# SludgePhD/Compeg

Hardware: AMD Instinct MI355X
Metric: Mpixels/s decoded (4K 4:2:2 restart-interval baseline JPEG -> RGBA8 in HBM) (higher is better)
Workload: dtype u32 bit-reader / i16 levels / f32 IDCT / u8 RGBA

## Files before the change

### compeg_amd/csrc/runtime.cpp

```cpp
#include "runtime.h"
#include "lab.h"

#include <hip/hip_runtime.h>

#include <algorithm>
#include <chrono>
#include <string>
#include <cstdio>
#include <cstdlib>
#include <condition_variable>
#include <cstring>
#include <mutex>
#include <thread>

namespace compeg {

Status hip_status(hipError_t e, const char *what)
{
    if (e == hipSuccess)
        return Status{};
    char buf[256];
    snprintf(buf, sizeof buf, "%s: %s", what, hipGetErrorString(e));
    return Status::error(COMPEG_E_HIP, buf);
}
// ... 323 lines not shown
}

}

}

using namespace compeg;

compeg_decoder::compeg_decoder() : scan(pinned_alloc, pinned_free)
{
    const unsigned hw = std::thread::hardware_concurrency();
    unsigned threads = hw >= 32 ? 8 : (hw >= 8 ? 4 : 1);
    bool asked = false;
    if (const char *e = getenv("COMPEG_SCAN_THREADS")) {
        threads = unsigned(std::max(1, std::min(16, atoi(e))));
        asked = true;
    }
    scan.set_threads(threads, !asked);
}

compeg_decoder::~compeg_decoder()
{
    if (last_stream || upload_pending)
        (void)hipStreamSynchronize(last_stream);
    if (upload_done)
        (void)hipEventDestroy(upload_done);
    if (decode_done)
        (void)hipEventDestroy(decode_done);
    if (gpu)
        compeg_gpu_release(gpu);
}

Status compeg_decoder::preprocess_on_device(const ImageData &img, hipStream_t stream, uint32_t &nwords,
                                            uint32_t &nstarts, uint32_t &span, bool &fell_back, size_t blob_bytes,
                                            const BlobWriter &before_submit)
{
    fell_back = false;
    if (img.scan_len > 0xfffffff0u) {
        fell_back = true;
        return Status{};
    }
    const uint32_t len = uint32_t(img.scan_len), expected = img.metadata.total_restart_intervals;
    uint32_t slots = 1;
    while (slots < expected)
        slots <<= 1;
    const uint32_t ntiles = scan_tiles(len);
    size_t total = 64;
    auto take = [&](size_t bytes) {
        const size_t at = total;
        total += align_up(bytes, 256);
        return at;
    };
    const size_t o_res = 0, o_desc = take(sizeof(ScanDesc)), o_blob = take(before_submit ? blob_bytes : 0),
                 o_raw = take(size_t(len) + 64), o_ts = take(size_t(ntiles) * kScanTileStateBytes + 32),
                 o_st = take(size_t(slots) * 4), o_w = take(size_t(len) + len / 3 + 64);
    CG_TRY(scan_arena.reserve(total + kStreamSlackBytes));
    CG_TRY(raw_stage.reserve(o_raw + len + 64));
    uint8_t *da = static_cast<uint8_t *>(scan_arena.ptr), *hs = static_cast<uint8_t *>(raw_stage.ptr);
    ScanDesc s;
    s.raw = da + o_raw;
    s.len = len;
    s.ntiles = ntiles;
    s.slots = slots;
    s.tile_state = reinterpret_cast<uint32_t *>(da + o_ts);
    s.starts_out = reinterpret_cast<uint32_t *>(da + o_st);
    s.words_out = da + o_w;
    s.result = reinterpret_cast<uint32_t *>(da + o_res);
    dev_words = da + o_w;
    dev_starts = da + o_st;
    EnqueueTrace trace;
    memset(hs, 0, o_blob);
    if (before_submit)
        CG_TRY(before_submit(hs + o_blob, da + o_blob, &s.patch_nwords, &s.patch_nstarts));
    memcpy(hs + o_desc, &s, sizeof s);
    const size_t piece = scan.threads() > 1 ? size_t(len) + 1 : size_t(640u << 10);
    for (size_t at = 0; at < len || at == 0; at += piece) {
        const size_t n = std::min<size_t>(piece, len - at);
        scan.copy(hs + o_raw + at, img.scan_data() + at, n);
        const size_t from = at ? o_raw + at : 0;
        if (pull_copies())
            CG_HIP(launch_pull(da + from, hs + from, o_raw + at + n - from, stream));
        else
            CG_HIP(hipMemcpyAsync(da + from, hs + from, o_raw + at + n - from, hipMemcpyHostToDevice, stream));
        if (len == 0)
            break;
    }
    trace.mark("  stage_and_copy");
    CG_HIP(launch_scan(reinterpret_cast<const ScanDesc *>(da + o_desc), 1, ntiles, stream));
    CG_TRY(scan_result.reserve(16));
    uint32_t *res = static_cast<uint32_t *>(scan_result.ptr);
    scan_result_dev = da + o_res;
    deferred_expected = expected;
    if (!before_submit)
        CG_HIP(hipMemcpyAsync(res, scan_result_dev, 16, hipMemcpyDeviceToHost, stream));
    trace.mark("submit");
    if (before_submit) {
        const uint64_t most_words = (uint64_t(len) + 3u * uint64_t(expected)) / 4u + 1u;
        const uint64_t avg = expected ? (most_words + expected - 1) / expected : most_words;
        span = uint32_t(std::min<uint64_t>(2 * avg * kWave + 64, 0x7fffffffu));
        nwords = nstarts = 0;
        deferred_check = true;
        return Status{};
    }
    CG_HIP(hipStreamSynchronize(stream));
    trace.mark("sync");
    CG_TRY(check_scan_result(fell_back));
    if (fell_back)
        return Status{};
    nwords = res[2];
    nstarts = std::min(res[0], slots);
    const uint64_t avg = expected ? (uint64_t(nwords) + expected - 1) / expected : nwords;
    span = uint32_t(std::min<uint64_t>(2 * avg * kWave + 64, 0x7fffffffu));
    return Status{};
}

Status compeg_decoder::check_scan_result(bool &fell_back)
{
    const uint32_t *res = static_cast<const uint32_t *>(scan_result.ptr);
    fell_back = (res[3] & 1u) != 0u;
    if (!fell_back && res[0] != deferred_expected) {
        char msg[128];
        snprintf(msg, sizeof msg, "restart interval count mismatch: counted %u, expected %u", res[0],
                 deferred_expected);
        warning = msg;
    }
    return Status{};
}

Status compeg_decoder::finish_deferred(const ImageData &img, hipStream_t stream)
{
    if (!deferred_check)
        return Status{};
    deferred_check = false;
    bool fell_back = false;
    CG_TRY(check_scan_result(fell_back));
    if (!fell_back)
        return Status{};
    const bool keep = device_preprocess;
    device_preprocess = false;
    Status st = enqueue(img, stream, nullptr, false);
    device_preprocess = keep;
    CG_TRY(st);
    CG_HIP(hipStreamSynchronize(stream));
    return Status{};
}

Status compeg_decoder::enqueue(const ImageData &img, hipStream_t stream, bool *changed, bool may_defer)
{
    EnqueueTrace trace;
    const auto t_enter = std::chrono::steady_clock::now();
    stage_times = compeg_stage_times{0.0, 0.0, 0.0};
    double preprocess_us = 0.0;
    struct Closer {
        compeg_decoder *self;
        std::chrono::steady_clock::time_point t0;
        const double *pre;
        ~Closer()
        {
            self->stage_times.preprocess_us = *pre;
            self->stage_times.enqueue_writes_us = EnqueueTrace::us_since(t0) - *pre;
        }
    } closer{this, t_enter, &preprocess_us};
    CG_HIP(hipSetDevice(gpu->device));
    warning.clear();

    if (!decode_done)
        CG_HIP(hipEventCreateWithFlags(&decode_done, hipEventDisableTiming));
    if (decode_pending && stream != last_stream)
        CG_HIP(hipStreamWaitEvent(stream, decode_done, 0));

    bool realloc_out = false;
    if (img.width > out_w || img.height > out_h || !out.ptr) {
// ... 260 lines not shown
            CG_TRY(ensure_walk_tables());
            CG_HIP(launch_coop_422(reinterpret_cast<const ImageDesc *>(db), 1, md.total_restart_intervals, coop, stream));
            last_kernel = COMPEG_KERNEL_COOP_TEAM;
        } else if (use_stream_kernel(plan, md.total_restart_intervals, 1)) {
            const uint64_t mcus = std::max<uint64_t>(1u, uint64_t(md.total_restart_intervals) * std::max(1u, uint32_t(md.restart_interval)));
            const StreamPlan sp = plan_stream(md.total_restart_intervals, 1, staged_lut_entries(img),
                                              uint32_t((img.scan_len / 4u + mcus - 1u) / mcus), true);
            CG_HIP(launch_fused_stream(reinterpret_cast<const ImageDesc *>(db), 1, md.total_restart_intervals, sp, stream));
            last_kernel = COMPEG_KERNEL_FUSED_STREAM;
        } else if (use_pair_kernel(md.total_restart_intervals, 1)) {
            CG_HIP(launch_pair_422(reinterpret_cast<const ImageDesc *>(db), 1, md.total_restart_intervals,
                                   plan, stream));
            last_kernel = COMPEG_KERNEL_PAIR;
        } else {
            CG_HIP(launch_fused_422(reinterpret_cast<const ImageDesc *>(db), 1, md.total_restart_intervals,
                                    plan, stream, false, md.restart_interval == 1u));
            last_kernel = COMPEG_KERNEL_FUSED;
        }
        coefficients_valid = false;
    } else {
        last_kernel = COMPEG_KERNEL_SPLIT;
        CG_HIP(launch_entropy(reinterpret_cast<const ImageDesc *>(db), 1, md.total_restart_intervals,
                              plan, stream));
        CG_HIP(launch_idct_composite(reinterpret_cast<const ImageDesc *>(db), 1, total_dus, stream));
        coefficients_valid = true;
    }
    if (deferred_check)
        CG_HIP(hipMemcpyAsync(scan_result.ptr, scan_result_dev, 16, hipMemcpyDeviceToHost, stream));
    if (!may_defer) {
        CG_HIP(hipEventRecord(decode_done, stream));
        decode_pending = true;
    }
    trace.mark("launch");
    return Status{};
}

Status compeg::ScanBuffer::process_on_gpu(compeg_gpu *gpu, const uint8_t *scan, size_t len,
                                          uint32_t expected)
{
    if (len > 0xfffffff0u)
        return Status::error(COMPEG_E_INVALID_ARG, "scan segment too large");
    CG_HIP(hipSetDevice(gpu->device));
    uint32_t slots = 1;
    while (slots < expected)
        slots <<= 1;
    const uint32_t ntiles = scan_tiles(uint32_t(len));
    DeviceBuffer arena, descbuf;
    size_t total = 64;
    auto take = [&](size_t bytes) {
        const size_t at = total;
        total += align_up(bytes, 256);
        return at;
    };
    const size_t o_raw = take(len + 64), o_ts = take(size_t(ntiles) * kScanTileStateBytes + 32),
                 o_st = take(size_t(slots) * 4), o_w = take(len + len / 3 + 64), o_res = take(kScanResultBytes);
    CG_TRY(arena.reserve(total));
    CG_TRY(descbuf.reserve(sizeof(ScanDesc)));
    uint8_t *da = static_cast<uint8_t *>(arena.ptr);
    CG_HIP(hipMemset(da, 0, total));
    if (len)
        CG_HIP(hipMemcpy(da + o_raw, scan, len, hipMemcpyHostToDevice));
    ScanDesc s;
    s.raw = da + o_raw;
    s.len = uint32_t(len);
    s.ntiles = ntiles;
    s.slots = slots;
    s.tile_state = reinterpret_cast<uint32_t *>(da + o_ts);
    s.starts_out = reinterpret_cast<uint32_t *>(da + o_st);
    s.words_out = da + o_w;
    s.result = reinterpret_cast<uint32_t *>(da + o_res);
    CG_HIP(hipMemcpy(descbuf.ptr, &s, sizeof s, hipMemcpyHostToDevice));
    CG_HIP(launch_scan(static_cast<const ScanDesc *>(descbuf.ptr), 1, ntiles, gpu->stream));
    CG_HIP(hipStreamSynchronize(gpu->stream));
    uint32_t res[4];
    CG_HIP(hipMemcpy(res, da + o_res, 16, hipMemcpyDeviceToHost));
    if (res[3] & 1u)
        return process(scan, len, expected);
    const size_t out_cap = ((len + len / 3 + 3) / 4) * 4;
    if (!words_.reserve(out_cap + 8) || !starts_.reserve(size_t(slots) * 4))
        return Status::error(COMPEG_E_HIP, "out of host memory in ScanBuffer");
    nwords_ = res[2];
    nstarts_ = std::min(res[0], slots);
    if (nwords_)
        CG_HIP(hipMemcpy(words_.data, da + o_w, nwords_ * 4, hipMemcpyDeviceToHost));
    if (nstarts_)
        CG_HIP(hipMemcpy(starts_.data, da + o_st, nstarts_ * 4, hipMemcpyDeviceToHost));
    if (res[0] != expected) {
        char msg[128];
        snprintf(msg, sizeof msg, "restart interval count mismatch: counted %u, expected %u", res[0], expected);
        return Status::error(COMPEG_E_COUNT_MISMATCH, msg);
    }
    return Status{};
}

hipError_t shared_copy_streams(int device, std::vector<hipStream_t> &out)
{
    static std::mutex m;
    static std::vector<hipStream_t> pool[64];
    std::lock_guard<std::mutex> lock(m);
    if (device < 0 || device >= 64)
        return hipErrorInvalidDevice;
    while (pool[device].size() < 4) {
        hipStream_t c = nullptr;
        const hipError_t e = hipStreamCreateWithFlags(&c, hipStreamNonBlocking);
        if (e != hipSuccess)
            return e;
        pool[device].push_back(c);
    }
    out = pool[device];
    return hipSuccess;
}

compeg_batch::~compeg_batch()
{
    (void)hipStreamSynchronize(last_stream);
    if (gpu)
        (void)hipStreamSynchronize(gpu->stream);
    for (hipStream_t c : copy_streams)
        (void)hipStreamSynchronize(c);
    for (hipEvent_t e : events)
        (void)hipEventDestroy(e);
    if (decode_done)
        (void)hipEventDestroy(decode_done);
    if (gpu)
        compeg_gpu_release(gpu);
}

namespace {

constexpr const char *kLayoutBoundExceeded = "layout bound exceeded";
// ... 492 lines not shown
        const uint8_t *host;
        size_t bytes, dev;
    };
    std::vector<Run> runs;
    std::vector<size_t> run_of(n, 0);
    for (size_t i = 0; i < n; i++) {
        bool joins = false;
        if (!runs.empty() && pinned[i] && pinned[i - 1]) {
            const Run &r = runs.back();
            const uint8_t *end = r.host + r.bytes;
            const bool one_allocation = alloc[i].base && alloc[i].base == alloc[i - 1].base && alloc[i].end == alloc[i - 1].end &&
                                        src[i].bytes + src[i].len <= alloc[i].end && r.host >= alloc[i].base;
            joins = group_of(i) == group_of(r.first) && src[i].bytes >= end && size_t(src[i].bytes - end) <= kMaxGap &&
                    (src[i].bytes == end || one_allocation) && size_t(src[i].bytes - r.host) + src[i].len <= kMaxRunBytes;
        }
        if (joins) {
            runs.back().last = i;
            runs.back().bytes = size_t(src[i].bytes - runs.back().host) + src[i].len;
        } else {
            runs.push_back(Run{i, i, src[i].bytes, src[i].len, 0});
        }
        run_of[i] = runs.size() - 1;
    }

    struct Layout {
        size_t sent, tables, tile_state, starts, words;
        size_t staged;
        size_t tile_cap, slot_cap;
    };
    std::vector<Layout> lay(n);
    size_t total = 0;
    auto take = [&](size_t bytes) {
        const size_t at = total;
        total += align_up(bytes, 256);
        return at;
    };
    const size_t o_results = take(n * kScanResultBytes);
    constexpr size_t kUnparsedTablesCap = size_t(32) << 10;
    size_t tables_bytes = 0;
    for (size_t i = 0; i < n; i++) {
        lay[i].tables = tables_bytes;
        tables_bytes += align_up(given ? table_blob_bytes(*given[i]) : kUnparsedTablesCap, 256);
    }
    const size_t o_tables = take(tables_bytes);
    size_t staged_total = align_up(tables_bytes, 256);
    for (Run &r : runs)
        r.dev = take(64 + align_up(r.bytes + 64, 16)) + 64;
    for (size_t i = 0; i < n; i++) {
        Layout &L = lay[i];
        const size_t len = src[i].len;
        L.tables += o_tables;
        L.sent = runs[run_of[i]].dev + size_t(src[i].bytes - runs[run_of[i]].host);
        L.tile_cap = scan_tiles(uint32_t(len));
        L.tile_state = take(L.tile_cap * kScanTileStateBytes + 32);
        L.slot_cap = ScanBuffer::start_slots(src[i].intervals);
        L.starts = take(L.slot_cap * 4);
        L.words = take(len + len / 3 + 64);
        L.staged = staged_total;
        staged_total += align_up(len + 64, 256);
    }
    CG_TRY(scan_arena.reserve(total + kStreamSlackBytes));
    CG_TRY(scan_descs.reserve(n * sizeof(ScanDesc) + 256));
    hipStream_t st = gpu->stream;
    CG_TRY(dev_descs.reserve(n * sizeof(ImageDesc) + 256));
    CG_HIP(shared_copy_streams(gpu->device, copy_streams));
    uint8_t *da = static_cast<uint8_t *>(scan_arena.ptr);
    CG_HIP(hipMemsetAsync(da + o_results, 0, n * kScanResultBytes, st));
    CG_TRY(stage.reserve((any_pageable ? staged_total : align_up(tables_bytes, 256)) + 256));
    uint8_t *hs = static_cast<uint8_t *>(stage.ptr);
    const double t_layout = ms_since();

    std::vector<std::atomic<uint8_t>> staged_ready(n), parsed_ready(n);
    for (size_t i = 0; i < n; i++) {
        staged_ready[i].store(pinned[i], std::memory_order_relaxed);
        parsed_ready[i].store(given ? 1 : 0, std::memory_order_relaxed);
    }
    unsigned nthreads = threads > 0 ? unsigned(threads) : std::min(16u, std::max(1u, std::thread::hardware_concurrency()));
    nthreads = unsigned(std::min<size_t>(nthreads, std::max<size_t>(n, 1)));
    std::atomic<size_t> next_image{0};
    std::atomic<int> hip_error{int(hipSuccess)};
    std::atomic<bool> failed{false};
    std::vector<Status> results(n);
    const int device = gpu->device;
    auto prepare_images = [&] {
        for (;;) {
            const size_t i = next_image.fetch_add(1, std::memory_order_relaxed);
            if (i >= n)
                return;
            if (!given) {
                images[i] = parse(i, results[i]);
                if (!images[i] || table_blob_bytes(*images[i]) > kUnparsedTablesCap) {
                    if (images[i] && results[i].ok())
                        results[i] = Status::error(COMPEG_E_INVALID_ARG, kLayoutBoundExceeded);
                    images[i] = nullptr;
                    failed.store(true, std::memory_order_relaxed);
                }
                parsed_ready[i].store(1, std::memory_order_release);
            }
            if (!pinned[i]) {
                memcpy(hs + lay[i].staged, src[i].bytes, src[i].len);
                staged_ready[i].store(1, std::memory_order_release);
            }
            if (images[i])
                write_tables(hs + (lay[i].tables - o_tables), *images[i]);
        }
    };
    std::vector<ScanDesc> sd(n);
// ... 140 lines not shown
        CG_HIP(hipMemcpyAsync(res.data(), da + o_results, n * kScanResultBytes, hipMemcpyDeviceToHost, st));

        max_tiles = 0;
        max_intervals = max_dus = max_l2 = max_span = 0;
        algorithmic_bytes = pixels = 0;
        size_t out_total = 0;
        bool all_covered = true;
        for (size_t i = 0; i < n; i++) {
            const ImageData &img = *images[i];
            out_total += align_up(output_bytes(img.width, img.height), 256);
            max_tiles = std::max(max_tiles, sd[i].ntiles);
            max_intervals = std::max(max_intervals, img.metadata.total_restart_intervals);
            max_dus = std::max(max_dus, img.total_dus());
            max_l2 = std::max<uint32_t>(max_l2, staged_lut_entries(img));
            pixels += uint64_t(img.width) * img.height;
            all_covered = all_covered && item_of(img).covered;
        }
        note_batch_properties(images.data(), n);
        size_t ac_total = 0, dc_total = 0;
        for (size_t i = 0; i < n && generic_layout; i++) {
            ac_total += size_t(images[i]->total_dus()) * kRetained * 2;
            dc_total += size_t(images[i]->total_dus()) * 4;
        }
        if (generic_layout) {
            CG_TRY(ac.reserve(ac_total + 256));
            CG_TRY(dc.reserve(dc_total + 256));
        }
        bool fresh_out = false;
        CG_TRY(out.reserve(out_total + 256, &fresh_out));
        if (fresh_out || !all_covered)
            CG_HIP(hipMemsetAsync(out.ptr, 0, out.capacity, st));
        CG_HIP(hipStreamSynchronize(st));
        const double t_arrived = ms_since();
        last_stream = st;

        descs.assign(n, ImageDesc{});
        out_offset.assign(n, 0);
        host_fallbacks = 0;
        size_t out_at = 0, ac_at = 0, dc_at = 0;
        for (size_t i = 0; i < n; i++) {
            const Layout &L = lay[i];
            const uint32_t *r = &res[i * (kScanResultBytes / 4)];
            uint32_t nwords = r[2], nstarts = std::min(r[0], sd[i].slots), span = r[4];
            const bool ends_earlier = (r[3] & 2u) != 0u && images[i]->scan_end_deferred;
            if (ends_earlier) {
                Status ps;
                const ImageData *again = reparse ? reparse(i, ps) : nullptr;
                if (!again)
                    return ps.ok() ? Status::error(COMPEG_E_MALFORMED, "entropy-coded segment ends early") : ps;
                images[i] = again;
            }
            const ImageData &img = *images[i];
            const uint32_t expected = img.metadata.total_restart_intervals;
            if ((r[3] & 1u) || ends_earlier) {
                ScanBuffer sb;
                Status s = sb.process(img.scan_data(), img.scan_len, expected);
                if (!s.ok() && s.code != COMPEG_E_COUNT_MISMATCH)
                    return s;
                nwords = uint32_t(sb.nwords());
                nstarts = uint32_t(sb.nstarts());
                if (nwords)
                    CG_HIP(hipMemcpy(da + L.words, sb.words(), size_t(nwords) * 4, hipMemcpyHostToDevice));
                if (nstarts)
                    CG_HIP(hipMemcpy(da + L.starts, sb.starts(), size_t(nstarts) * 4, hipMemcpyHostToDevice));
                span = max_wave_span(sb.starts(), nstarts, nwords, expected);
                host_fallbacks++;
            }
            ImageDesc &d = descs[i];
            fill_desc(img, d);
            d.l1 = reinterpret_cast<const uint16_t *>(da + L.tables);
            d.l2 = reinterpret_cast<const uint16_t *>(da + L.tables + COMPEG_HUFFMAN_L1_BYTES);
            d.words = reinterpret_cast<const uint32_t *>(da + L.words);
            d.starts = reinterpret_cast<const uint32_t *>(da + L.starts);
            d.nwords = nwords;
            d.nstarts = nstarts;
            d.ac = generic_layout ? reinterpret_cast<int16_t *>(static_cast<uint8_t *>(ac.ptr) + ac_at) : nullptr;
            d.dc = generic_layout ? reinterpret_cast<int32_t *>(static_cast<uint8_t *>(dc.ptr) + dc_at) : nullptr;
            ac_at += size_t(img.total_dus()) * kRetained * 2;
            dc_at += size_t(img.total_dus()) * 4;
            out_offset[i] = out_at;
            d.out = static_cast<uint8_t *>(out.ptr) + out_at;
            out_at += align_up(output_bytes(img.width, img.height), 256);
            d.out_w = img.width;
            d.out_h = img.height;
            d.out_pitch = output_pitch(img.width);
            d.out_alloc_h = output_rows(img.height);
            max_span = std::max(max_span, span);
            if (i == 0) {
                coop_r = img.metadata.restart_interval;
                coop_spans = CoopSpans{};
            }
            if (!d.coop_ok || img.metadata.restart_interval != coop_r) {
                coop_r = 0;
            } else {
                coop_spans_max(coop_spans, coop_spans_estimate(span, coop_r, true));
            }
            algorithmic_bytes += 4ull * nwords + 4ull * expected + COMPEG_METADATA_BYTES +
                                 COMPEG_HUFFMAN_L1_BYTES + img.l2.size() * 2 + 4ull * img.width * img.height;
        }
        CG_TRY(make_walk_tables(gpu->stream, n));
        CG_HIP(hipStreamSynchronize(gpu->stream));
        count = n;
        decodes_timed = 0;
        if (trace_on) {
            size_t direct = 0;
            for (size_t i = 0; i < n; i++)
                direct += pinned[i];
// ... 232 lines not shown
```

### compeg_amd/csrc/scan_kernels.h

```cpp
#pragma once

#include <hip/hip_runtime_api.h>

#include <cstddef>
#include <cstdint>

namespace compeg {

struct ScanDesc {
    const uint8_t *raw;
    uint32_t len;
    uint32_t ntiles;
    uint32_t slots;
    uint32_t *tile_state;
    uint32_t *starts_out;
    uint8_t *words_out;
    uint32_t expected = 0;
    uint32_t *result;
    uint32_t *patch_nwords = nullptr;
    uint32_t *patch_nstarts = nullptr;
};

constexpr size_t kScanTileStateBytes = 20;
uint32_t scan_tiles(uint32_t len);
hipError_t launch_pull(void *dst, const void *pinned_src, size_t bytes, hipStream_t stream);
hipError_t launch_pull3(void *const dst[3], const void *const pinned_src[3], const size_t bytes[3], hipStream_t stream);
hipError_t launch_scan(const ScanDesc *descs, uint32_t images, uint32_t max_tiles, hipStream_t stream,
                       bool with_span = false);
constexpr size_t kScanResultBytes = 32;

}
```

### compeg_amd/csrc/scan_kernels.hip

```cpp
#include <hip/hip_runtime.h>

#include <algorithm>

#include "scan_kernels.h"

namespace compeg {
namespace {

constexpr uint32_t kTileBytes = 4096;
constexpr uint32_t kThreads = 256;
constexpr uint32_t kBytesPerThread = kTileBytes / kThreads;
constexpr uint32_t kMaxLookBack = 512;

struct Chunk {
    uint32_t w[4];
    uint32_t n;
    uint32_t kept;
    uint32_t marker;
    uint32_t foreign;
};

__device__ __forceinline__ uint32_t byte_of(const uint32_t (&w)[4], uint32_t i)
{
    return (w[i >> 2] >> ((i & 3u) * 8u)) & 0xffu;
}

__device__ uint32_t ff_run_before_slow(const ScanDesc &d, uint32_t pos)
{
    uint32_t r = 0;
    while (r < pos && r < kMaxLookBack && d.raw[pos - 1 - r] == 0xff)
        r++;
    if (r >= kMaxLookBack && r < pos)
        atomicOr(&d.result[3], 1u);
    return r;
}

__device__ __forceinline__ void load_classify(const ScanDesc &d, uint32_t g, Chunk &c)
{
    c.n = g < d.len ? min(kBytesPerThread, d.len - g) : 0u;
    c.kept = c.marker = c.foreign = 0u;
    c.w[0] = c.w[1] = c.w[2] = c.w[3] = 0u;
    uint32_t next = 0;
    if (c.n) {
        const uintptr_t addr = reinterpret_cast<uintptr_t>(d.raw) + g;
        const uint32_t mis = uint32_t(addr & 3u);
        const uint32_t *src = reinterpret_cast<const uint32_t *>(addr - mis);
        uint32_t a[5];
        for (int i = 0; i < 5; i++)
            a[i] = src[i];
        for (int i = 0; i < 4; i++)
            c.w[i] = mis ? (a[i] >> (mis * 8u)) | (a[i + 1] << (32u - mis * 8u)) : a[i];
        next = mis ? (a[4] >> (mis * 8u)) & 0xffu : a[4] & 0xffu;
        if (g + 16u >= d.len)
            next = 0;
    }
    uint32_t r = 0;
    if (c.n && g > 0 && d.raw[g - 1] == 0xff)
        r = ff_run_before_slow(d, g);

    uint32_t F = 0, Z = 0, R = 0;
    for (int k = 0; k < 4; k++) {
        const uint32_t x = c.w[k], nx = ~x, rx = (x ^ 0xd0d0d0d0u) & 0xf8f8f8f8u;
        const uint32_t zf = ~(((nx & 0x7f7f7f7fu) + 0x7f7f7f7fu) | nx) & 0x80808080u;
        const uint32_t zz = ~(((x & 0x7f7f7f7fu) + 0x7f7f7f7fu) | x) & 0x80808080u;
        const uint32_t zr = ~(((rx & 0x7f7f7f7fu) + 0x7f7f7f7fu) | rx) & 0x80808080u;
        F |= (((zf >> 7) * 0x00204081u) >> 21 & 0xfu) << (4 * k);
        Z |= (((zz >> 7) * 0x00204081u) >> 21 & 0xfu) << (4 * k);
        R |= (((zr >> 7) * 0x00204081u) >> 21 & 0xfu) << (4 * k);
    }
    const uint32_t valid = c.n >= 16u ? 0xffffu : ((1u << c.n) - 1u);
    F &= valid;
    c.foreign = ((F << 1) | (r ? 1u : 0u)) & ~F & ~Z & ~R & valid;
    const uint32_t starts = F & ~(F << 1);
    uint32_t even_starts = starts & 0x5555u, odd_starts = starts & 0xaaaau;
    if ((r & 1u) && (F & 1u)) {
        even_starts &= ~1u;
        odd_starts |= 1u;
    }
    (void)odd_starts;
    const uint32_t in_even_runs = F & ~(F + even_starts);
    const uint32_t lead = (in_even_runs & 0x5555u) | (F & ~in_even_runs & 0xaaaau);
    const uint32_t partner = ((lead << 1) | (r & 1u)) & 0xffffu;
    const uint32_t next_zero = ((Z >> 1) | ((next == 0u ? 1u : 0u) << 15)) & 0xffffu;
    const uint32_t remaining = d.len - g;
    const uint32_t has_next = remaining > 16u ? 0xffffu : (remaining >= 2u ? ((1u << (remaining - 1u)) - 1u) : 0u);
    c.kept = ((~F & ~partner) | (lead & next_zero & has_next)) & valid;
    c.marker = lead & ~next_zero & has_next & valid;
}

struct Stretch {
    uint32_t markers, head, words, tail, kept;
};

static_assert(sizeof(Stretch) == kScanTileStateBytes, "tile_state stride");

__device__ __forceinline__ Stretch stretch_none() { return Stretch{0u, 0u, 0u, 0u, 0u}; }

__device__ __forceinline__ Stretch join(const Stretch &l, const Stretch &r)
{
    Stretch o;
    o.kept = l.kept + r.kept;
    o.markers = l.markers + r.markers;
    const bool lm = l.markers != 0u, rm = r.markers != 0u;
    o.head = lm ? l.head : l.head + r.head;
    o.tail = rm ? r.tail : l.tail + r.tail;
    o.words = l.words + r.words + ((lm && rm) ? (l.tail + r.head + 3u) / 4u : 0u);
    return o;
}

__device__ __forceinline__ Stretch stretch_shfl_up(const Stretch &x, uint32_t o)
{
    return Stretch{__shfl_up(x.markers, o), __shfl_up(x.head, o), __shfl_up(x.words, o), __shfl_up(x.tail, o),
                   __shfl_up(x.kept, o)};
}

struct Cursor {
    uint32_t interval, start_word, bytes;
};

__device__ __forceinline__ Cursor cursor_behind(const Stretch &before)
{
    if (before.markers == 0u)
        return Cursor{0u, 0u, before.kept};
    return Cursor{before.markers, (before.head + 3u) / 4u + before.words, before.tail};
}

__device__ __forceinline__ Stretch stretch_of(const Chunk &c)
{
    Stretch s;
    s.kept = __popc(c.kept);
    s.markers = __popc(c.marker);
    s.words = 0u;
    if (s.markers == 0u) {
        s.head = s.tail = s.kept;
        return s;
    }
    const uint32_t first = uint32_t(__ffs(int(c.marker))) - 1u, last = 31u - uint32_t(__clz(int(c.marker)));
    s.head = __popc(c.kept & ((1u << first) - 1u));
    s.tail = __popc(c.kept & ~((2u << last) - 1u));
    uint32_t prev = first;
    for (uint32_t mk = c.marker & (c.marker - 1u); mk; mk &= mk - 1u) {
        const uint32_t i = uint32_t(__ffs(int(mk))) - 1u;
        s.words += (__popc(c.kept & ((1u << i) - 1u) & ~((2u << prev) - 1u)) + 3u) / 4u;
        prev = i;
    }
    return s;
}

__device__ __forceinline__ Stretch block_exclusive_scan(const Stretch &mine, Stretch *lds, Stretch &total)
{
    const uint32_t lane = threadIdx.x & 63u, wave = threadIdx.x >> 6;
    Stretch x = mine;
    for (uint32_t o = 1; o < 64; o <<= 1) {
        const Stretch y = stretch_shfl_up(x, o);
        if (lane >= o)
            x = join(y, x);
    }
    if (lane == 63)
        lds[wave] = x;
    __syncthreads();
    Stretch before = stretch_none();
    total = stretch_none();
    for (uint32_t w = 0; w < kThreads / 64u; w++) {
        const Stretch t = lds[w];
        if (w < wave)
            before = join(before, t);
        total = join(total, t);
    }
    __syncthreads();
    Stretch prev = stretch_shfl_up(x, 1);
    if (lane == 0)
        prev = stretch_none();
    return join(before, prev);
}

__global__ void __launch_bounds__(kThreads) count_kernel(const ScanDesc *descs)
{
    __shared__ Stretch lds[kThreads / 64u];
    const ScanDesc &d = descs[blockIdx.y];
    const uint32_t tile = blockIdx.x;
    if (tile >= d.ntiles)
        return;
    const uint32_t g = tile * kTileBytes + threadIdx.x * kBytesPerThread;
    Chunk c;
    load_classify(d, g, c);
    if (c.foreign)
        atomicOr(&d.result[3], 2u);
    Stretch total;
    block_exclusive_scan(stretch_of(c), lds, total);
    if (threadIdx.x == 0)
        reinterpret_cast<Stretch *>(d.tile_state)[tile] = total;
}

__global__ void __launch_bounds__(kThreads) tile_scan_kernel(const ScanDesc *descs)
{
    __shared__ Stretch lds[kThreads / 64u];
    const ScanDesc &d = descs[blockIdx.x];
    Stretch *tiles = reinterpret_cast<Stretch *>(d.tile_state);
    Stretch carry = stretch_none();
    for (uint32_t base = 0; base < d.ntiles; base += kThreads) {
        const uint32_t i = base + threadIdx.x;
        const Stretch mine = i < d.ntiles ? tiles[i] : stretch_none();
        Stretch total;
        const Stretch before = block_exclusive_scan(mine, lds, total);
        if (i < d.ntiles)
            tiles[i] = join(carry, before);
        carry = join(carry, total);
    }
    if (threadIdx.x == 0) {
        const uint32_t count = carry.markers + 1u;
        const Cursor end = cursor_behind(carry);
        const uint32_t words = end.start_word + (end.bytes + 3u) / 4u;
        d.result[0] = count;
        d.result[1] = carry.kept;
        d.result[2] = words;
        if (d.patch_nwords)
            *d.patch_nwords = words;
        if (d.patch_nstarts)
            *d.patch_nstarts = min(count, d.slots);
        d.starts_out[0] = 0u;
    }
}

constexpr uint32_t kOutStageBytes = kTileBytes + 3u * (kTileBytes / 2u) + 32u;

__global__ void __launch_bounds__(kThreads) emit_kernel(const ScanDesc *descs)
{
    __shared__ Stretch lds[kThreads / 64u];
    __shared__ uint32_t span[2];
    __shared__ __attribute__((aligned(16))) uint8_t stage[kOutStageBytes];
    const ScanDesc &d = descs[blockIdx.y];
    const uint32_t tile = blockIdx.x;
    if (tile >= d.ntiles)
        return;
    const uint32_t count = d.result[0];
    const uint32_t g = tile * kTileBytes + threadIdx.x * kBytesPerThread;
    Chunk c;
    load_classify(d, g, c);
    Stretch total;
    const Stretch in_tile = block_exclusive_scan(stretch_of(c), lds, total);
    Cursor at = cursor_behind(join(reinterpret_cast<const Stretch *>(d.tile_state)[tile], in_tile));

    const uint32_t zero_dwords = min((total.kept + 3u * total.markers + 11u) / 4u, kOutStageBytes / 4u);
    for (uint32_t i = threadIdx.x; i < zero_dwords; i += kThreads)
        reinterpret_cast<uint32_t *>(stage)[i] = 0u;
    uint32_t end = at.start_word * 4u + at.bytes;
    if (threadIdx.x == 0)
        span[0] = end;
    __syncthreads();
    const uint32_t lo = span[0];
    const uint32_t origin = lo & ~3u;
    if (c.kept == 0xffffu) {
        const uint32_t o = end - origin, sh = (o & 3u) * 8u;
        uint32_t *dst = reinterpret_cast<uint32_t *>(stage) + (o >> 2);
        if (sh == 0u) {
            for (int k = 0; k < 4; k++)
                dst[k] = c.w[k];
        } else {
            atomicOr(&dst[0], c.w[0] << sh);
            for (int k = 1; k < 4; k++)
                atomicOr(&dst[k], (c.w[k] << sh) | (c.w[k - 1] >> (32u - sh)));
            atomicOr(&dst[4], c.w[3] >> (32u - sh));
        }
        end += 16u;
    } else {
        for (uint32_t i = 0; i < kBytesPerThread; i++) {
            if (c.kept >> i & 1u) {
                stage[end - origin] = uint8_t(byte_of(c.w, i));
                at.bytes++;
                end++;
            } else if (c.marker >> i & 1u) {
                at.interval++;
                at.start_word += (at.bytes + 3u) / 4u;
                at.bytes = 0u;
                end = at.start_word * 4u;
                if (at.interval + d.slots >= count)
                    d.starts_out[at.interval & (d.slots - 1u)] = at.start_word;
            }
        }
    }
    if (c.n && (g + c.n == d.len || threadIdx.x == kThreads - 1)) {
        span[1] = (g + c.n == d.len) ? (end + 3u) & ~3u : end;
    }
    __syncthreads();
    const uint32_t hi = span[1];
    if (hi <= lo)
        return;
    const uint32_t body_lo = (lo + 3u) & ~3u, body_hi = hi & ~3u;
    if (body_lo >= body_hi) {
        for (uint32_t i = lo + threadIdx.x; i < hi; i += kThreads)
            d.words_out[i] = stage[i - origin];
        return;
    }
    if (threadIdx.x < body_lo - lo)
        d.words_out[lo + threadIdx.x] = stage[lo - origin + threadIdx.x];
    if (threadIdx.x < hi - body_hi)
        d.words_out[body_hi + threadIdx.x] = stage[body_hi - origin + threadIdx.x];
    uint32_t *out32 = reinterpret_cast<uint32_t *>(d.words_out);
    const uint32_t *stage32 = reinterpret_cast<const uint32_t *>(stage);
    for (uint32_t i = body_lo / 4u + threadIdx.x; i < body_hi / 4u; i += kThreads)
        out32[i] = stage32[i - origin / 4u];
}

__global__ void __launch_bounds__(kThreads) span_kernel(const ScanDesc *descs)
{
    __shared__ uint32_t best;
    const ScanDesc &d = descs[blockIdx.x];
    const uint32_t nstarts = min(d.result[0], d.slots), nwords = d.result[2], intervals = d.expected;
    if (threadIdx.x == 0)
        best = 0u;
    __syncthreads();
    uint32_t mine = 0;
    for (uint32_t first = threadIdx.x * 64u; first < intervals; first += kThreads * 64u) {
        const uint32_t lo = first < nstarts ? d.starts_out[first] : 0u;
        const uint32_t after = first + 64u;
        const uint32_t hi = (after < intervals && after < nstarts) ? d.starts_out[after] : nwords;
        if (hi > lo)
            mine = max(mine, hi - lo);
    }
    atomicMax(&best, mine);
    __syncthreads();
    if (threadIdx.x == 0)
        d.result[4] = best;
}

typedef uint32_t PullVec __attribute__((ext_vector_type(4)));

__global__ void __launch_bounds__(kThreads) pull_kernel(PullVec *__restrict__ dst, const PullVec *__restrict__ src,
                                                        uint32_t n16)
{
    for (uint32_t i = blockIdx.x * kThreads + threadIdx.x; i < n16; i += gridDim.x * kThreads)
        dst[i] = __builtin_nontemporal_load(src + i);
}

struct PullSegs {
    PullVec *dst[3];
    const PullVec *src[3];
    uint32_t n16[3];
};
__global__ void __launch_bounds__(kThreads) pull3_kernel(PullSegs segs)
{
#pragma unroll
    for (int k = 0; k < 3; k++)
        for (uint32_t i = blockIdx.x * kThreads + threadIdx.x; i < segs.n16[k]; i += gridDim.x * kThreads)
            segs.dst[k][i] = __builtin_nontemporal_load(segs.src[k] + i);
}

}

hipError_t launch_pull3(void *const dst[3], const void *const pinned_src[3], const size_t bytes[3], hipStream_t stream)
{
    PullSegs segs{};
    size_t most = 0;
    for (int k = 0; k < 3; k++) {
        const size_t n16 = (bytes[k] + 15) / 16;
        if (n16 > 0xffffffffu)
            return hipErrorInvalidValue;
        segs.dst[k] = static_cast<PullVec *>(dst[k]);
        segs.src[k] = static_cast<const PullVec *>(pinned_src[k]);
        segs.n16[k] = uint32_t(n16);
        most = std::max(most, n16);
    }
    if (most == 0)
        return hipSuccess;
    const uint32_t blocks = uint32_t(std::min<size_t>((most + kThreads - 1) / kThreads, 48));
    hipLaunchKernelGGL(pull3_kernel, dim3(blocks), dim3(kThreads), 0, stream, segs);
    return hipGetLastError();
}

hipError_t launch_pull(void *dst, const void *pinned_src, size_t bytes, hipStream_t stream)
{
    const size_t n16 = (bytes + 15) / 16;
    if (n16 == 0)
        return hipSuccess;
    if (n16 > 0xffffffffu)
        return hipErrorInvalidValue;
    const uint32_t blocks = uint32_t(std::min<size_t>((n16 + kThreads - 1) / kThreads, 48));
    hipLaunchKernelGGL(pull_kernel, dim3(blocks), dim3(kThreads), 0, stream, static_cast<PullVec *>(dst),
                       static_cast<const PullVec *>(pinned_src), uint32_t(n16));
    return hipGetLastError();
}

uint32_t scan_tiles(uint32_t len)
{
    return (len + kTileBytes - 1) / kTileBytes;
}

hipError_t launch_scan(const ScanDesc *descs, uint32_t images, uint32_t max_tiles, hipStream_t stream, bool with_span)
{
    if (images == 0)
        return hipSuccess;
    if (max_tiles) {
        hipLaunchKernelGGL(count_kernel, dim3(max_tiles, images), dim3(kThreads), 0, stream, descs);
    }
    hipLaunchKernelGGL(tile_scan_kernel, dim3(images), dim3(kThreads), 0, stream, descs);
    if (max_tiles) {
        hipLaunchKernelGGL(emit_kernel, dim3(max_tiles, images), dim3(kThreads), 0, stream, descs);
    }
    if (with_span)
        hipLaunchKernelGGL(span_kernel, dim3(images), dim3(kThreads), 0, stream, descs);
    return hipGetLastError();
}

}
```

Measured before the change: 772,100.

## Replace three-pass marker scan with single-pass decoupled look-back scan kernel

Replaces the count/tile-scan/emit three-kernel pipeline with one kernel. Each workgroup takes a dynamic ticket, classifies four tiles, publishes its aggregate with epoch-tagged flags, resolves its prefix by decoupled look-back over predecessors, then emits unstuffed words and restart starts directly. This removes two launches and the second read and classify pass over the scan data. The cost is spin-waiting, a bounded poll count that falls back to the CPU path, and a new wrap flag that reruns the old three-pass scan when restart slots overflow.

```diff
diff --git a/compeg_amd/csrc/runtime.cpp b/compeg_amd/csrc/runtime.cpp
--- a/compeg_amd/csrc/runtime.cpp
+++ b/compeg_amd/csrc/runtime.cpp
@@ -399,7 +399,7 @@
         return at;
     };
     const size_t o_res = 0, o_desc = take(sizeof(ScanDesc)), o_blob = take(before_submit ? blob_bytes : 0),
-                 o_raw = take(size_t(len) + 64), o_ts = take(size_t(ntiles) * kScanTileStateBytes + 32),
+                 o_raw = take(size_t(len) + 64), o_ts = take(scan_state_bytes(ntiles)),
                  o_st = take(size_t(slots) * 4), o_w = take(size_t(len) + len / 3 + 64);
     CG_TRY(scan_arena.reserve(total + kStreamSlackBytes));
     CG_TRY(raw_stage.reserve(o_raw + len + 64));
@@ -464,7 +464,7 @@
 Status compeg_decoder::check_scan_result(bool &fell_back)
 {
     const uint32_t *res = static_cast<const uint32_t *>(scan_result.ptr);
-    fell_back = (res[3] & 1u) != 0u;
+    fell_back = (res[3] & kScanFlagsGaveUp) != 0u;
     if (!fell_back && res[0] != deferred_expected) {
         char msg[128];
         snprintf(msg, sizeof msg, "restart interval count mismatch: counted %u, expected %u", res[0],
@@ -831,7 +831,7 @@
         total += align_up(bytes, 256);
         return at;
     };
-    const size_t o_raw = take(len + 64), o_ts = take(size_t(ntiles) * kScanTileStateBytes + 32),
+    const size_t o_raw = take(len + 64 + 16) + (reinterpret_cast<uintptr_t>(scan) & 15u), o_ts = take(scan_state_bytes(ntiles)),
                  o_st = take(size_t(slots) * 4), o_w = take(len + len / 3 + 64), o_res = take(kScanResultBytes);
     CG_TRY(arena.reserve(total));
     CG_TRY(descbuf.reserve(sizeof(ScanDesc)));
@@ -853,8 +853,16 @@
     CG_HIP(hipStreamSynchronize(gpu->stream));
     uint32_t res[4];
     CG_HIP(hipMemcpy(res, da + o_res, 16, hipMemcpyDeviceToHost));
-    if (res[3] & 1u)
+    if (res[3] & (kScanFlagLongFfRun | kScanFlagWaitBound))
         return process(scan, len, expected);
+    if (res[3] & kScanFlagWrapped) {
+        CG_HIP(hipMemset(da + o_res, 0, kScanResultBytes));
+        CG_HIP(launch_scan_three_pass(static_cast<const ScanDesc *>(descbuf.ptr), 1, ntiles, gpu->stream));
+        CG_HIP(hipStreamSynchronize(gpu->stream));
+        CG_HIP(hipMemcpy(res, da + o_res, 16, hipMemcpyDeviceToHost));
+        if (res[3] & kScanFlagLongFfRun)
+            return process(scan, len, expected);
+    }
     const size_t out_cap = ((len + len / 3 + 3) / 4) * 4;
     if (!words_.reserve(out_cap + 8) || !starts_.reserve(size_t(slots) * 4))
         return Status::error(COMPEG_E_HIP, "out of host memory in ScanBuffer");
@@ -1453,7 +1461,7 @@
         L.tables += o_tables;
         L.sent = runs[run_of[i]].dev + size_t(src[i].bytes - runs[run_of[i]].host);
         L.tile_cap = scan_tiles(uint32_t(len));
-        L.tile_state = take(L.tile_cap * kScanTileStateBytes + 32);
+        L.tile_state = take(scan_state_bytes(uint32_t(L.tile_cap)));
         L.slot_cap = ScanBuffer::start_slots(src[i].intervals);
         L.starts = take(L.slot_cap * 4);
         L.words = take(len + len / 3 + 64);
@@ -1700,7 +1708,7 @@
             }
             const ImageData &img = *images[i];
             const uint32_t expected = img.metadata.total_restart_intervals;
-            if ((r[3] & 1u) || ends_earlier) {
+            if ((r[3] & kScanFlagsGaveUp) || ends_earlier) {
                 ScanBuffer sb;
                 Status s = sb.process(img.scan_data(), img.scan_len, expected);
                 if (!s.ok() && s.code != COMPEG_E_COUNT_MISMATCH)
diff --git a/compeg_amd/csrc/scan_algebra.h b/compeg_amd/csrc/scan_algebra.h
--- /dev/null
+++ b/compeg_amd/csrc/scan_algebra.h
@@ -0,0 +1,53 @@
+#pragma once
+
+#include <cstdint>
+
+#ifdef __HIP__
+#define CG_SCAN_FN __host__ __device__ __forceinline__
+#else
+#define CG_SCAN_FN inline
+#endif
+
+namespace compeg {
+
+struct Stretch {
+    uint32_t markers, head, words, tail, kept;
+};
+
+CG_SCAN_FN Stretch stretch_none() { return Stretch{0u, 0u, 0u, 0u, 0u}; }
+
+CG_SCAN_FN Stretch join(const Stretch &l, const Stretch &r)
+{
+    Stretch o;
+    o.kept = l.kept + r.kept;
+    o.markers = l.markers + r.markers;
+    const bool lm = l.markers != 0u, rm = r.markers != 0u;
+    o.head = lm ? l.head : l.head + r.head;
+    o.tail = rm ? r.tail : l.tail + r.tail;
+    o.words = l.words + r.words + ((lm && rm) ? (l.tail + r.head + 3u) / 4u : 0u);
+    return o;
+}
+
+struct Cursor {
+    uint32_t interval, start_word, bytes;
+};
+
+CG_SCAN_FN Cursor cursor_behind(const Stretch &before)
+{
+    if (before.markers == 0u)
+        return Cursor{0u, 0u, before.kept};
+    return Cursor{before.markers, (before.head + 3u) / 4u + before.words, before.tail};
+}
+
+constexpr uint32_t kScanGroupTiles = 4;
+constexpr uint32_t kScanGroupStateWords = 12;
+constexpr uint32_t kScanFlagTag = 0x80000000u;
+constexpr uint32_t kScanEpochMask = 0x1fffffffu;
+enum : uint32_t { kScanNothing = 0u, kScanAggregate = 1u, kScanPrefix = 2u, kScanGaveUp = 3u };
+CG_SCAN_FN uint32_t scan_flag_base(uint32_t epoch) { return kScanFlagTag | ((epoch & kScanEpochMask) << 2); }
+CG_SCAN_FN uint32_t scan_flag_state(uint32_t word, uint32_t base)
+{
+    return (word & ~3u) == base ? (word & 3u) : uint32_t(kScanNothing);
+}
+
+}
diff --git a/compeg_amd/csrc/scan_kernels.h b/compeg_amd/csrc/scan_kernels.h
--- a/compeg_amd/csrc/scan_kernels.h
+++ b/compeg_amd/csrc/scan_kernels.h
@@ -2,8 +2,11 @@
 
 #include <hip/hip_runtime_api.h>
 
+#include <algorithm>
 #include <cstddef>
 #include <cstdint>
+
+#include "scan_algebra.h"
 
 namespace compeg {
 
@@ -21,12 +24,24 @@
     uint32_t *patch_nstarts = nullptr;
 };
 
+constexpr uint32_t kScanFlagLongFfRun = 1u;
+constexpr uint32_t kScanFlagForeign = 2u;
+constexpr uint32_t kScanFlagWaitBound = 4u;
+constexpr uint32_t kScanFlagWrapped = 8u;
+constexpr uint32_t kScanFlagsGaveUp = kScanFlagLongFfRun | kScanFlagWaitBound | kScanFlagWrapped;
+
 constexpr size_t kScanTileStateBytes = 20;
+inline size_t scan_state_bytes(uint32_t ntiles)
+{
+    const size_t groups = (size_t(ntiles) + kScanGroupTiles - 1) / kScanGroupTiles;
+    return std::max(size_t(ntiles) * kScanTileStateBytes, groups * kScanGroupStateWords * 4) + 32;
+}
 uint32_t scan_tiles(uint32_t len);
 hipError_t launch_pull(void *dst, const void *pinned_src, size_t bytes, hipStream_t stream);
 hipError_t launch_pull3(void *const dst[3], const void *const pinned_src[3], const size_t bytes[3], hipStream_t stream);
 hipError_t launch_scan(const ScanDesc *descs, uint32_t images, uint32_t max_tiles, hipStream_t stream,
                        bool with_span = false);
+hipError_t launch_scan_three_pass(const ScanDesc *descs, uint32_t images, uint32_t max_tiles, hipStream_t stream);
 constexpr size_t kScanResultBytes = 32;
 
 }
diff --git a/compeg_amd/csrc/scan_kernels.hip b/compeg_amd/csrc/scan_kernels.hip
--- a/compeg_amd/csrc/scan_kernels.hip
+++ b/compeg_amd/csrc/scan_kernels.hip
@@ -1,6 +1,7 @@
 #include <hip/hip_runtime.h>
 
 #include <algorithm>
+#include <atomic>
 
 #include "scan_kernels.h"
 
@@ -88,41 +89,13 @@
     c.marker = lead & ~next_zero & has_next & valid;
 }
 
-struct Stretch {
-    uint32_t markers, head, words, tail, kept;
-};
 
 static_assert(sizeof(Stretch) == kScanTileStateBytes, "tile_state stride");
-
-__device__ __forceinline__ Stretch stretch_none() { return Stretch{0u, 0u, 0u, 0u, 0u}; }
-
-__device__ __forceinline__ Stretch join(const Stretch &l, const Stretch &r)
-{
-    Stretch o;
-    o.kept = l.kept + r.kept;
-    o.markers = l.markers + r.markers;
-    const bool lm = l.markers != 0u, rm = r.markers != 0u;
-    o.head = lm ? l.head : l.head + r.head;
-    o.tail = rm ? r.tail : l.tail + r.tail;
-    o.words = l.words + r.words + ((lm && rm) ? (l.tail + r.head + 3u) / 4u : 0u);
-    return o;
-}
 
 __device__ __forceinline__ Stretch stretch_shfl_up(const Stretch &x, uint32_t o)
 {
     return Stretch{__shfl_up(x.markers, o), __shfl_up(x.head, o), __shfl_up(x.words, o), __shfl_up(x.tail, o),
                    __shfl_up(x.kept, o)};
-}
-
-struct Cursor {
-    uint32_t interval, start_word, bytes;
-};
-
-__device__ __forceinline__ Cursor cursor_behind(const Stretch &before)
-{
-    if (before.markers == 0u)
-        return Cursor{0u, 0u, before.kept};
-    return Cursor{before.markers, (before.head + 3u) / 4u + before.words, before.tail};
 }
 
 __device__ __forceinline__ Stretch stretch_of(const Chunk &c)
@@ -224,23 +197,10 @@
 
 constexpr uint32_t kOutStageBytes = kTileBytes + 3u * (kTileBytes / 2u) + 32u;
 
-__global__ void __launch_bounds__(kThreads) emit_kernel(const ScanDesc *descs)
-{
-    __shared__ Stretch lds[kThreads / 64u];
-    __shared__ uint32_t span[2];
-    __shared__ __attribute__((aligned(16))) uint8_t stage[kOutStageBytes];
-    const ScanDesc &d = descs[blockIdx.y];
-    const uint32_t tile = blockIdx.x;
-    if (tile >= d.ntiles)
-        return;
-    const uint32_t count = d.result[0];
-    const uint32_t g = tile * kTileBytes + threadIdx.x * kBytesPerThread;
-    Chunk c;
-    load_classify(d, g, c);
-    Stretch total;
-    const Stretch in_tile = block_exclusive_scan(stretch_of(c), lds, total);
-    Cursor at = cursor_behind(join(reinterpret_cast<const Stretch *>(d.tile_state)[tile], in_tile));
-
+template <bool kOnePass>
+__device__ __forceinline__ void emit_tile(const ScanDesc &d, const Chunk &c, uint32_t g, const Stretch &total, Cursor at,
+                                          uint32_t count, uint32_t *span, uint8_t *stage)
+{
     const uint32_t zero_dwords = min((total.kept + 3u * total.markers + 11u) / 4u, kOutStageBytes / 4u);
     for (uint32_t i = threadIdx.x; i < zero_dwords; i += kThreads)
         reinterpret_cast<uint32_t *>(stage)[i] = 0u;
@@ -274,7 +234,7 @@
                 at.start_word += (at.bytes + 3u) / 4u;
                 at.bytes = 0u;
                 end = at.start_word * 4u;
-                if (at.interval + d.slots >= count)
+                if (kOnePass ? at.interval < d.slots : at.interval + d.slots >= count)
                     d.starts_out[at.interval & (d.slots - 1u)] = at.start_word;
             }
         }
@@ -300,6 +260,217 @@
     const uint32_t *stage32 = reinterpret_cast<const uint32_t *>(stage);
     for (uint32_t i = body_lo / 4u + threadIdx.x; i < body_hi / 4u; i += kThreads)
         out32[i] = stage32[i - origin / 4u];
+}
+
+__global__ void __launch_bounds__(kThreads) emit_kernel(const ScanDesc *descs)
+{
+    __shared__ Stretch lds[kThreads / 64u];
+    __shared__ uint32_t span[2];
+    __shared__ __attribute__((aligned(16))) uint8_t stage[kOutStageBytes];
+    const ScanDesc &d = descs[blockIdx.y];
+    const uint32_t tile = blockIdx.x;
+    if (tile >= d.ntiles)
+        return;
+    const uint32_t count = d.result[0];
+    const uint32_t g = tile * kTileBytes + threadIdx.x * kBytesPerThread;
+    Chunk c;
+    load_classify(d, g, c);
+    Stretch total;
+    const Stretch in_tile = block_exclusive_scan(stretch_of(c), lds, total);
+    const Cursor at = cursor_behind(join(reinterpret_cast<const Stretch *>(d.tile_state)[tile], in_tile));
+    emit_tile<false>(d, c, g, total, at, count, span, stage);
+}
+
+typedef __attribute__((address_space(1))) uint32_t GlobalU32;
+typedef __attribute__((address_space(1))) unsigned long long GlobalU64;
+
+constexpr uint32_t kMaxPolls = 1u << 18;
+
+__device__ __forceinline__ void publish(uint32_t *group_state, uint32_t at_word, const Stretch &v, uint32_t flag)
+{
+    GlobalU32 *s = (GlobalU32 *)group_state;
+    GlobalU64 *p = (GlobalU64 *)(s + at_word);
+    __hip_atomic_store(p, uint64_t(v.markers) | uint64_t(v.head) << 32, __ATOMIC_RELAXED, __HIP_MEMORY_SCOPE_AGENT);
+    __hip_atomic_store(p + 1, uint64_t(v.words) | uint64_t(v.tail) << 32, __ATOMIC_RELAXED, __HIP_MEMORY_SCOPE_AGENT);
+    __hip_atomic_store(s + at_word + 4, v.kept, __ATOMIC_RELAXED, __HIP_MEMORY_SCOPE_AGENT);
+    asm volatile("s_waitcnt vmcnt(0)" ::: "memory");
+    __hip_atomic_store(s + 5, flag, __ATOMIC_RELAXED, __HIP_MEMORY_SCOPE_AGENT);
+}
+
+__device__ __forceinline__ void publish_gave_up(uint32_t *group_state, uint32_t base)
+{
+    __hip_atomic_store((GlobalU32 *)group_state + 5, base | kScanGaveUp, __ATOMIC_RELAXED, __HIP_MEMORY_SCOPE_AGENT);
+}
+
+__device__ __forceinline__ Stretch load_published(const uint32_t *group_state, uint32_t at_word)
+{
+    const GlobalU32 *s = (const GlobalU32 *)group_state;
+    const GlobalU64 *p = (const GlobalU64 *)(s + at_word);
+    const uint64_t a = __hip_atomic_load(p, __ATOMIC_RELAXED, __HIP_MEMORY_SCOPE_AGENT);
+    const uint64_t b = __hip_atomic_load(p + 1, __ATOMIC_RELAXED, __HIP_MEMORY_SCOPE_AGENT);
+    const uint32_t k = __hip_atomic_load(s + at_word + 4, __ATOMIC_RELAXED, __HIP_MEMORY_SCOPE_AGENT);
+    return Stretch{uint32_t(a), uint32_t(a >> 32), uint32_t(b), uint32_t(b >> 32), k};
+}
+
+__device__ __forceinline__ Stretch stretch_shfl(const Stretch &x, int lane)
+{
+    return Stretch{__shfl(x.markers, lane), __shfl(x.head, lane), __shfl(x.words, lane), __shfl(x.tail, lane),
+                   __shfl(x.kept, lane)};
+}
+
+__device__ bool look_back(const uint32_t *states, uint32_t group, uint32_t base, Stretch &before)
+{
+    const int lane = int(threadIdx.x & 63u);
+    before = stretch_none();
+    for (int nearest = int(group) - 1;; nearest -= 64) {
+        const int p = nearest - 63 + lane;
+        const GlobalU32 *flag = (const GlobalU32 *)(states + size_t(p < 0 ? 0 : p) * kScanGroupStateWords) + 5;
+        uint32_t state = kScanAggregate;
+        for (uint32_t polls = 0;; polls++) {
+            if (p >= 0)
+                state = scan_flag_state(__hip_atomic_load(flag, __ATOMIC_RELAXED, __HIP_MEMORY_SCOPE_AGENT), base);
+            if (__all(state != kScanNothing))
+                break;
+            if (polls >= kMaxPolls)
+                return false;
+            __builtin_amdgcn_s_sleep(8);
+        }
+        __builtin_amdgcn_fence(__ATOMIC_ACQUIRE, "wavefront");
+        if (__any(state == kScanGaveUp))
+            return false;
+        const unsigned long long has_prefix = __ballot(p >= 0 && state == kScanPrefix);
+        const int from = has_prefix ? 63 - __clzll((long long)has_prefix) : 0;
+        Stretch x = stretch_none();
+        if (p >= 0 && lane >= from)
+            x = load_published(states + size_t(p) * kScanGroupStateWords, state == kScanPrefix ? 6u : 0u);
+        for (uint32_t o = 1; o < 64; o <<= 1) {
+            const Stretch y = stretch_shfl_up(x, o);
+            if (lane >= int(o))
+                x = join(y, x);
+        }
+        before = join(stretch_shfl(x, 63), before);
+        if (has_prefix)
+            return true;
+        if (nearest < 64)
+            return false;
+    }
+}
+
+__device__ __forceinline__ void write_result(const ScanDesc &d, const Stretch &all)
+{
+    const uint32_t count = all.markers + 1u;
+    const Cursor end = cursor_behind(all);
+    const uint32_t words = end.start_word + (end.bytes + 3u) / 4u;
+    d.result[0] = count;
+    d.result[1] = all.kept;
+    d.result[2] = words;
+    if (d.patch_nwords)
+        *d.patch_nwords = words;
+    if (d.patch_nstarts)
+        *d.patch_nstarts = min(count, d.slots);
+}
+
+__global__ void __launch_bounds__(kThreads) scan_kernel(const ScanDesc *descs, uint32_t groups_per_image,
+                                                        uint32_t total_groups, uint32_t epoch)
+{
+    __shared__ Stretch lds[kThreads / 64u];
+    __shared__ Stretch before_shared;
+    __shared__ uint32_t span[2];
+    __shared__ uint32_t ticket, resolved;
+    __shared__ __attribute__((aligned(16))) uint8_t stage[kOutStageBytes];
+    if (threadIdx.x == 0) {
+        uint32_t *counter = descs[0].result + 5;
+        const uint32_t t = atomicAdd(counter, 1u);
+        if (t + 1u == total_groups)
+            atomicExch(counter, 0u);
+        ticket = t;
+    }
+    __syncthreads();
+    const uint32_t image = ticket / groups_per_image, group = ticket % groups_per_image;
+    const ScanDesc &d = descs[image];
+    const uint32_t ngroups = (d.ntiles + kScanGroupTiles - 1u) / kScanGroupTiles;
+    if (d.ntiles == 0u || d.len >= kScanFlagTag) {
+        if (group == 0u && threadIdx.x == 0) {
+            if (d.ntiles == 0u) {
+                write_result(d, stretch_none());
+                d.starts_out[0] = 0u;
+            } else {
+                atomicOr(&d.result[3], kScanFlagWaitBound);
+            }
+        }
+        return;
+    }
+    if (group >= ngroups)
+        return;
+
+    Chunk c[kScanGroupTiles];
+    const uint32_t g0 = group * kScanGroupTiles * kTileBytes + threadIdx.x * kBytesPerThread;
+    uint32_t foreign = 0;
+#pragma unroll
+    for (uint32_t k = 0; k < kScanGroupTiles; k++) {
+        load_classify(d, g0 + k * kTileBytes, c[k]);
+        foreign |= c[k].foreign;
+    }
+    if (foreign)
+        atomicOr(&d.result[3], kScanFlagForeign);
+    Stretch aggregate = stretch_none();
+#pragma unroll
+    for (uint32_t k = 0; k < kScanGroupTiles; k++) {
+        Stretch total;
+        block_exclusive_scan(stretch_of(c[k]), lds, total);
+        aggregate = join(aggregate, total);
+    }
+
+    uint32_t *mine = d.tile_state + size_t(group) * kScanGroupStateWords;
+    const uint32_t base = scan_flag_base(epoch);
+    if (threadIdx.x < 64u) {
+        Stretch before = stretch_none();
+        bool ok = true;
+        if (group == 0u) {
+            if (threadIdx.x == 0)
+                publish(mine, 6u, aggregate, base | kScanPrefix);
+        } else {
+            if (threadIdx.x == 0)
+                publish(mine, 0u, aggregate, base | kScanAggregate);
+            ok = look_back(d.tile_state, group, base, before);
+            if (threadIdx.x == 0) {
+                if (ok)
+                    publish(mine, 6u, join(before, aggregate), base | kScanPrefix);
+                else
+                    publish_gave_up(mine, base);
+            }
+        }
+        if (threadIdx.x == 0) {
+            before_shared = before;
+            resolved = ok ? 1u : 0u;
+        }
+    }
+    __syncthreads();
+    if (!resolved) {
+        if (threadIdx.x == 0)
+            atomicOr(&d.result[3], kScanFlagWaitBound);
+        return;
+    }
+    Stretch before = before_shared;
+    if (group + 1u == ngroups && threadIdx.x == 0) {
+        const Stretch all = join(before, aggregate);
+        write_result(d, all);
+        if (all.markers + 1u > d.slots)
+            atomicOr(&d.result[3], kScanFlagWrapped);
+    }
+    if (group == 0u && threadIdx.x == 0)
+        d.starts_out[0] = 0u;
+
+#pragma unroll
+    for (uint32_t k = 0; k < kScanGroupTiles; k++) {
+        if (group * kScanGroupTiles + k >= d.ntiles)
+            break;
+        Stretch total;
+        const Stretch in_tile = block_exclusive_scan(stretch_of(c[k]), lds, total);
+        emit_tile<true>(d, c[k], g0 + k * kTileBytes, total, cursor_behind(join(before, in_tile)), 0u, span, stage);
+        before = join(before, total);
+        __syncthreads();
+    }
 }
 
 __global__ void __launch_bounds__(kThreads) span_kernel(const ScanDesc *descs)
@@ -390,6 +561,26 @@
 {
     if (images == 0)
         return hipSuccess;
+    static std::atomic<uint32_t> launches{0};
+    uint32_t epoch;
+    do
+        epoch = (launches.fetch_add(1, std::memory_order_relaxed) + 1u) & kScanEpochMask;
+    while (epoch == 0u);
+    const uint64_t groups_per_image = std::max<uint64_t>(1, (uint64_t(max_tiles) + kScanGroupTiles - 1) / kScanGroupTiles);
+    const uint64_t total_groups = groups_per_image * images;
+    if (total_groups > 0x7fffffffu)
+        return hipErrorInvalidValue;
+    hipLaunchKernelGGL(scan_kernel, dim3(uint32_t(total_groups)), dim3(kThreads), 0, stream, descs,
+                       uint32_t(groups_per_image), uint32_t(total_groups), epoch);
+    if (with_span)
+        hipLaunchKernelGGL(span_kernel, dim3(images), dim3(kThreads), 0, stream, descs);
+    return hipGetLastError();
+}
+
+hipError_t launch_scan_three_pass(const ScanDesc *descs, uint32_t images, uint32_t max_tiles, hipStream_t stream)
+{
+    if (images == 0)
+        return hipSuccess;
     if (max_tiles) {
         hipLaunchKernelGGL(count_kernel, dim3(max_tiles, images), dim3(kThreads), 0, stream, descs);
     }
@@ -397,8 +588,6 @@
     if (max_tiles) {
         hipLaunchKernelGGL(emit_kernel, dim3(max_tiles, images), dim3(kThreads), 0, stream, descs);
     }
-    if (with_span)
-        hipLaunchKernelGGL(span_kernel, dim3(images), dim3(kThreads), 0, stream, descs);
     return hipGetLastError();
 }
 
```

Result: no change. 771,800 (median of 2 runs) (-0.0%).
